# mmailhos/vectorlite

Measured on AMD Instinct MI355X. Metric: flat-cosine QPS @ N=10M dim=384 k=10; achieved HBM GB/s vs peak, higher is better.
Workload: dtype f32; 1 GPU; flat cosine single-query search, N=10000000, dim=384, k=10; rows=10000000, dim=384, k=10, metric=cosine, parallelism=1 GPU

## Files before the change

### vectorlite_amd/csrc/kernels.hip

```cpp
#include "kernels.hpp"
#include "device_common.hpp"
#include "scan_stream.hpp"
#include "score_bound.hpp"

#include <math.h>
#include <stdlib.h>
#include <string.h>

#include <mutex>
#include <tuple>
#include <type_traits>

namespace vl {
using namespace dev;
static_assert(BOUND_COSINE == COSINE && BOUND_EUCLIDEAN == EUCLIDEAN && BOUND_MANHATTAN == MANHATTAN && BOUND_DOT == DOT,
              "score_bound.hpp carries the metric codes of kernels.hpp");
namespace {

template <typename K, typename C>
__global__ __launch_bounds__(1024) void k_merge_lists(const C* __restrict__ lists, int n_lists, size_t in_stride_q,
                                                      C* __restrict__ out, size_t out_stride_q)
{
    constexpr int NW = 16;
    __shared__ C sh[NW * WAVE];
// ... 367 lines not shown
    {
        const uint32_t first = blockIdx.y * QB;
        q64 += (size_t)first * dim;
        out += (size_t)first * gridDim.x * KP;
        n_q = n_q - first < (uint32_t)QB ? n_q - first : (uint32_t)QB;
    }

    for (uint32_t idx = threadIdx.x; idx < QB * LD4; idx += 256) {
        const uint32_t qi = idx / LD4, j = idx % LD4;
        f32x4 z = {0.0f, 0.0f, 0.0f, 0.0f};
        qs[qi][j] = qi < n_q ? load_q4(q64 + (size_t)qi * dim, j, dim) : z;
    }
    __syncthreads();

    const uint32_t n_steps = (n + RPS - 1) / RPS;
    const uint32_t n_waves = gridDim.x * 4;

    TopList<float> L[QB];
    uint32_t n_buf[QB];
#pragma unroll
    for (int qi = 0; qi < QB; ++qi) {
        L[qi].init();
        n_buf[qi] = 0;
    }
    auto flush = [&](int qi) {
        float fk = -INFINITY;
        uint32_t fp = POS_SENTINEL;
        asm volatile("" : "+v"(fk));
        if ((uint32_t)lane < n_buf[qi]) {
            const Cand32 e = cbuf[wave][qi][lane];
            fk = e.key;
            fp = e.pos;
        }
        sort64_reversed<float>(fk, fp);
        L[qi].merge_reversed(fk, fp);
        n_buf[qi] = 0;
    };

    for (uint32_t s = blockIdx.x * 4 + wave; s < n_steps; s += n_waves) {
        const uint32_t row = s * RPS + g;
        const bool valid = row < n;
        const uint32_t r = valid ? row : n - 1;
        const f32x4* p = slab + (size_t)r * LD4 + c;
        f32x4 x[VPL];
#pragma unroll
        for (int j = 0; j < VPL; ++j) x[j] = __builtin_nontemporal_load(p + G * j);
        float inv = 1.0f;
        if (METRIC == COSINE) inv = inv_norm[r];
#pragma unroll
        for (int qi = 0; qi < QB; ++qi) {
            float a = 0.0f;
#pragma unroll
            for (int j = 0; j < VPL; ++j) a = acc4<METRIC>(a, x[j], qs[qi][c + G * j]);
            a = group_reduce<G>(a);
#ifndef VL_DBG_K3_NOINSERT
            {
                const float key = scan_key<METRIC>(a, inv);
                const bool cand = valid && c == 0 && (uint32_t)qi < n_q && better<float>(key, row, L[qi].thr_key, L[qi].thr_pos);
                const unsigned long long m = __ballot(cand);
                if (m != 0ull) {
                    const uint32_t slot = n_buf[qi] + __builtin_amdgcn_mbcnt_hi((uint32_t)(m >> 32), __builtin_amdgcn_mbcnt_lo((uint32_t)m, 0u));
                    if (cand) {
                        Cand32 e;
                        e.key = key;
                        e.pos = row;
                        cbuf[wave][qi][slot] = e;
                    }
                    n_buf[qi] += (uint32_t)__popcll(m);
                    if (n_buf[qi] > (uint32_t)(WAVE - RPS)) flush(qi);
                }
            }
#else
            if (scan_key<METRIC>(a, inv) == 12345.678f) L[qi].pos = row;
#endif
            __builtin_amdgcn_sched_barrier(0);
        }
    }

#pragma unroll
    for (int qi = 0; qi < QB; ++qi) {
        if ((uint32_t)qi < n_q) {
            if (n_buf[qi]) flush(qi);
            block_merge<float, Cand32, 4>(L[qi], sh);
            if (wave == 0) {
                Cand32 e;
                e.key = L[qi].key;
                e.pos = L[qi].pos;
                out[((size_t)qi * gridDim.x + blockIdx.x) * KP + lane] = e;
            }
            __syncthreads();
        }
    }
}

constexpr int RESCORE_CH = 96;

template <int METRIC, int NTHREADS>
__device__ __forceinline__ void rescore_rows(const double* __restrict__ master, const double* __restrict__ q64,
                                             uint32_t dim, const uint32_t* sh_pos, int n_rows,
                                             double (*tile)[RESCORE_CH + 1], double* qtile, Acc64<METRIC>& A)
{
    constexpr int PER = (KP * RESCORE_CH + NTHREADS - 1) / NTHREADS;
    constexpr int PF = (NTHREADS >= 1024) ? 4 : 1;
    const int tid = threadIdx.x;
    A.init();
    if (n_rows <= 0) return;
    for (uint32_t g0 = 0; g0 < dim; g0 += PF * RESCORE_CH) {
        double pre[PF][PER];
        double qpre[PF];
#pragma unroll
        for (int p = 0; p < PF; ++p) {
            const uint32_t c0 = g0 + p * RESCORE_CH;
#pragma unroll
            for (int i = 0; i < PER; ++i) {
                int idx = tid + i * NTHREADS;
                idx = idx < KP * RESCORE_CH ? idx : KP * RESCORE_CH - 1;
                int r = idx / RESCORE_CH;
                r = r < n_rows ? r : n_rows - 1;
                uint32_t col = c0 + (uint32_t)(idx % RESCORE_CH);
                col = col < dim ? col : dim - 1;
                pre[p][i] = master[(size_t)sh_pos[r] * dim + col];
            }
            {
                uint32_t col = c0 + (uint32_t)(tid % RESCORE_CH);
                col = col < dim ? col : dim - 1;
                qpre[p] = q64[col];
            }
        }
#pragma unroll
        for (int p = 0; p < PF; ++p) {
            const uint32_t c0 = g0 + p * RESCORE_CH;
            if (c0 >= dim) break;
            const uint32_t cw = (dim - c0) < (uint32_t)RESCORE_CH ? (dim - c0) : (uint32_t)RESCORE_CH;
            __syncthreads();
#pragma unroll
            for (int i = 0; i < PER; ++i) {
                const int idx = tid + i * NTHREADS;
                if (idx < KP * RESCORE_CH) tile[idx / RESCORE_CH][idx % RESCORE_CH] = pre[p][i];
            }
            if (tid < RESCORE_CH) qtile[tid] = qpre[p];
            __syncthreads();
            if (tid < n_rows) {
                uint32_t cc = 0;
                for (; cc + 8 <= cw; cc += 8) {
                    double xv[8], yv[8];
#pragma unroll
                    for (int t = 0; t < 8; ++t) {
                        xv[t] = tile[tid][cc + t];
                        yv[t] = qtile[cc + t];
                    }
#pragma unroll
                    for (int t = 0; t < 8; ++t) A.step(xv[t], yv[t]);
                }
                for (; cc < cw; ++cc) A.step(tile[tid][cc], qtile[cc]);
            }
        }
    }
}

#ifdef VL_DBG_STAMPS
__device__ unsigned long long vl_dbg_stamps[32];
#define VL_STAMP(i)                                                                  \
    do {                                                                             \
        if (threadIdx.x == 0 && blockIdx.x == 0) {                                   \
            vl_dbg_stamps[i] = __builtin_amdgcn_s_memrealtime();                     \
            vl_dbg_stamps[16 + (i)] = __builtin_amdgcn_s_memtime();  \
        }                                                                            \
    } while (0)
#else
#define VL_STAMP(i) do {} while (0)
#endif

constexpr int RP_CH = 48;
constexpr int RP_NCH = 8;
constexpr int RP_BW = RP_CH * RP_NCH;

template <int METRIC, int ROWS = KP, int NCH = RP_NCH>
struct RescoreLds {
    double tA[ROWS][RP_CH + 1];
    double tB[METRIC == COSINE ? ROWS : 1][RP_CH + 1];
    double qblk[RP_CH * NCH];
    double qq[METRIC == COSINE ? RP_CH * NCH : 1];
    double b[ROWS];
    double c;
};

template <int METRIC, int ROWS, int NTHREADS, int NCH = RP_NCH>
__device__ __forceinline__ void rescore_rows_par(const double* __restrict__ master, const double* __restrict__ q64,
                                                 uint32_t dim, const uint32_t* sh_pos, int n_rows,
                                                 RescoreLds<METRIC, ROWS, NCH>& S, Acc64<METRIC>& A,
                                                 const double (&q_first)[(RP_CH * NCH + NTHREADS - 1) / NTHREADS])
{
    constexpr int RP_PER = ROWS * RP_CH / NTHREADS;
    constexpr int BW = RP_CH * NCH;
    constexpr int QN = (BW + NTHREADS - 1) / NTHREADS;
    static_assert(ROWS * RP_CH % NTHREADS == 0 && ROWS <= WAVE, "tile elements divide evenly; one lane per row");
    const int tid = threadIdx.x;
    const int lane = tid & (WAVE - 1), wave = tid >> 6;
    A.init();
    if (n_rows <= 0) return;
    double acc = (METRIC == COSINE) ? 0.0 : -0.0;
    for (uint32_t g0 = 0; g0 < dim; g0 += BW) {
        double pre[NCH][RP_PER];
#pragma unroll
        for (int p = 0; p < NCH; ++p) {
            const uint32_t c0 = g0 + p * RP_CH;
#pragma unroll
            for (int i = 0; i < RP_PER; ++i) {
                const int idx = tid + i * NTHREADS;
                int r = idx / RP_CH;
                r = r < n_rows ? r : n_rows - 1;
                uint32_t col = c0 + (uint32_t)(idx % RP_CH);
                col = col < dim ? col : dim - 1;
                pre[p][i] = master[(size_t)sh_pos[r] * dim + col];
            }
        }
        double qv[QN];
#pragma unroll
        for (int j = 0; j < QN; ++j) {
            qv[j] = q_first[j];
            if (g0 != 0 && tid + j * NTHREADS < BW) {
                const uint32_t col = g0 + (uint32_t)(tid + j * NTHREADS);
                qv[j] = q64[col < dim ? col : dim - 1];
            }
        }
        VL_STAMP(4);
        __syncthreads();
#pragma unroll
        for (int j = 0; j < QN; ++j)
            if (tid + j * NTHREADS < BW) {
                S.qblk[tid + j * NTHREADS] = qv[j];
                if (METRIC == COSINE) S.qq[tid + j * NTHREADS] = qv[j] * qv[j];
            }
        __syncthreads();
        VL_STAMP(5);
#pragma unroll
        for (int p = 0; p < NCH; ++p) {
            const uint32_t c0 = g0 + p * RP_CH;
            if (c0 >= dim) break;
            const uint32_t cw = (dim - c0) < (uint32_t)RP_CH ? (dim - c0) : (uint32_t)RP_CH;
            if (p) __syncthreads();
#pragma unroll
            for (int i = 0; i < RP_PER; ++i) {
                const int idx = tid + i * NTHREADS;
                const int r = idx / RP_CH, cc = idx % RP_CH;
                const double x = pre[p][i], y = S.qblk[p * RP_CH + cc];
                if (METRIC == COSINE) {
                    S.tA[r][cc] = x * y;
                    S.tB[r][cc] = x * x;
                } else if (METRIC == EUCLIDEAN) {
                    const double d = x - y;
                    S.tA[r][cc] = d * d;
                } else if (METRIC == MANHATTAN) {
                    S.tA[r][cc] = fabs(x - y);
                } else {
                    S.tA[r][cc] = x * y;
                }
            }
            __syncthreads();
            if (wave == 0 || (METRIC == COSINE && wave == 1)) {
                if (lane < n_rows) {
                    const double* t = (wave == 0) ? &S.tA[lane][0] : &S.tB[METRIC == COSINE ? lane : 0][0];
                    uint32_t cc = 0;
                    for (; cc + 16 <= cw; cc += 16) {
                        double v[16];
#pragma unroll
                        for (int u = 0; u < 16; ++u) v[u] = t[cc + u];
#pragma unroll
                        for (int u = 0; u < 16; ++u) acc += v[u];
                    }
                    for (; cc < cw; ++cc) acc += t[cc];
                }
            } else if (METRIC == COSINE && wave == 2) {
                const double* t = &S.qq[p * RP_CH];
                uint32_t cc = 0;
                for (; cc + 16 <= cw; cc += 16) {
                    double v[16];
#pragma unroll
                    for (int u = 0; u < 16; ++u) v[u] = t[cc + u];
#pragma unroll
                    for (int u = 0; u < 16; ++u) acc += v[u];
                }
                for (; cc < cw; ++cc) acc += t[cc];
            }
            if (p == 0) VL_STAMP(6);
        }
    }
    VL_STAMP(7);
    __syncthreads();
    if (METRIC == COSINE) {
        if (wave == 1 && lane < ROWS) S.b[lane] = acc;
        if (wave == 2 && lane == 0) S.c = acc;
        __syncthreads();
        if (wave == 0) {
            A.a = acc;
            A.b = S.b[lane < ROWS ? lane : 0];
            A.c = S.c;
        }
    } else if (wave == 0) {
        A.a = acc;
    }
}


template <int METRIC>
__device__ __forceinline__ void rank_check_emit(double sc, uint32_t my_pos, float key64, int n_cand, uint32_t k, uint64_t n_rows,
                                                uint32_t ld, double R, double Q, double in_extra,
                                                SearchResultBlock* __restrict__ out, uint32_t seq, const ShardRecordSink& sink,
                                                uint32_t q_in_launch)
{
    const int lane = lane_id();
    const bool valid = lane < n_cand;
    const bool any_nan = __ballot(valid && sc != sc) != 0ull;
    int rank = 0;
    for (int j = 0; j < n_cand; ++j) {
        const double sj = read_lane(sc, j);
        const uint32_t pj = read_lane(my_pos, j);
        rank += (sj > sc || (sj == sc && pj < my_pos)) ? 1 : 0;
    }
    const uint32_t k_eff = (uint64_t)k < n_rows ? k : (uint32_t)n_rows;
    uint32_t flags = 0;
    if (any_nan) flags |= RESULT_HAS_NAN | RESULT_NEEDS_EXACT;
    if (n_rows <= (uint64_t)KP) {
        if ((uint64_t)n_cand < n_rows) flags |= RESULT_NEEDS_EXACT;
    } else {
        if (n_cand < KP) {
            flags |= RESULT_NEEDS_EXACT;
        } else {
            const double B = bound_for_key<METRIC>(key64, ld, R, Q, in_extra);
            const unsigned long long at_cut = __ballot(valid && rank == (int)k_eff - 1);
            double s_cut = 0.0;
            if (at_cut) s_cut = __shfl(sc, __ffsll((long long)at_cut) - 1);
            if (!at_cut || !(s_cut > B)) flags |= RESULT_NEEDS_EXACT;
        }
    }
    if (valid && rank < (int)k_eff) {
        out->pos[rank] = my_pos;
        out->score[rank] = sc;
    }
    if (lane == 0) {
        out->n_out = k_eff;
        out->flags = flags;
    }
    if (sink.cnt) {
        const uint32_t q = sink.q0 + q_in_launch;
        const uint32_t offered = (flags == 0u) ? (k_eff < sink.ks ? k_eff : sink.ks) : 0u;
        if (valid && (uint32_t)rank < offered) {
            const size_t e = (size_t)q * sink.ks + (uint32_t)rank;
            sink.score_bits[e] = (unsigned long long)__double_as_longlong(sc);
            sink.gpos[e] = sink.row_offset + (unsigned long long)my_pos;
            sink.ids[e] = sink.pos_to_id[my_pos];
        }
        if (lane == 0) sink.cnt[q] = offered;
    }
    VL_STAMP(9);
    if (seq) {
        __threadfence_system();
        if (lane == 0) __hip_atomic_store(&out->seq, seq, __ATOMIC_RELEASE, __HIP_MEMORY_SCOPE_SYSTEM);
    }
    VL_STAMP(10);
}

constexpr int BF_ROWS = 16;
#ifndef VL_BF_NCH
#define VL_BF_NCH 4
#endif
constexpr int BF_NCH = VL_BF_NCH;
template <int METRIC>
__global__ __launch_bounds__(256) void k_batch_rescore(const Cand32* __restrict__ lists, const double* __restrict__ master,
                                                       const double* __restrict__ q64, uint32_t dim, double* __restrict__ scores)
{
    const uint32_t q = blockIdx.x >> 2, quarter = blockIdx.x & 3u;
    __shared__ RescoreLds<METRIC, BF_ROWS, BF_NCH> rs;
    __shared__ uint32_t sh_pos[BF_ROWS];
    __shared__ int sh_n;
    const int tid = threadIdx.x, lane = tid & (WAVE - 1), wave = tid >> 6;
    const Cand32* mine = lists + (size_t)q * KP + quarter * BF_ROWS;
    q64 += (size_t)q * dim;
    constexpr int QN = (RP_CH * BF_NCH + 255) / 256;
    double q_first[QN];
#pragma unroll
    for (int j = 0; j < QN; ++j) {
        const uint32_t c = (uint32_t)(tid + j * 256);
        q_first[j] = q64[c < dim ? c : dim - 1];
    }
    if (wave == 0) {
        const uint32_t p = lane < BF_ROWS ? mine[lane].pos : POS_SENTINEL;
        if (lane < BF_ROWS) sh_pos[lane] = p;
        const unsigned long long real = __ballot(p != POS_SENTINEL);
        if (lane == 0) sh_n = __popcll(real);
    }
    __syncthreads();
    const int n_mine = sh_n;
    Acc64<METRIC> A;
    rescore_rows_par<METRIC, BF_ROWS, 256, BF_NCH>(master, q64, dim, sh_pos, n_mine, rs, A, q_first);
    if (wave == 0 && lane < BF_ROWS) scores[(size_t)q * KP + quarter * BF_ROWS + lane] = lane < n_mine ? A.score() : 0.0;
}

template <int METRIC>
__global__ __launch_bounds__(256) void k_batch_rank_emit(const Cand32* __restrict__ lists, const double* __restrict__ scores,
                                                         const double* __restrict__ q_norms, uint32_t nq, uint32_t ld,
                                                         uint64_t n_rows, uint32_t k, double R, double in_extra,
                                                         SearchResultBlock* __restrict__ out, ShardRecordSink sink)
{
    const int lane = lane_id();
    const uint32_t q = blockIdx.x * 4 + (threadIdx.x >> 6);
    if (q >= nq) return;
    const Cand32 e = lists[(size_t)q * KP + lane];
    const int n_cand = __popcll(__ballot(e.pos != POS_SENTINEL));
    const double sc = lane < n_cand ? scores[(size_t)q * KP + lane] : 0.0;
    rank_check_emit<METRIC>(sc, e.pos, read_lane(e.key, KP - 1), n_cand, k, n_rows, ld, R, q_norms[q], in_extra, out + q, 0u, sink, q);
}

template <int METRIC>
__global__ __launch_bounds__(1024) void k_merge_finalize(const Cand32* __restrict__ partials, int n_lists,
                                                         size_t list_stride_q, const double* __restrict__ master,
                                                         const double* __restrict__ q64,
                                                         const double* __restrict__ q_norms, uint32_t dim,
                                                         uint32_t ld, uint64_t n_rows, uint32_t k, double R,
                                                         double in_extra, SearchResultBlock* __restrict__ out,
                                                         uint32_t seq, ShardRecordSink sink)
{
    partials += (size_t)blockIdx.x * list_stride_q;
    q64 += (size_t)blockIdx.x * dim;
    out += blockIdx.x;
    const double Q = q_norms[blockIdx.x];
    constexpr int NW = 16;
    __shared__ Cand32 sh_lists[NW * WAVE];
    __shared__ RescoreLds<METRIC> rs;
    __shared__ uint32_t sh_pos[KP];
    __shared__ float sh_key[KP];
    __shared__ int sh_ncand;

    const int lane = lane_id();
    const int wave = threadIdx.x >> 6;

    VL_STAMP(0);
    TopList<float> L;
    double q_first[1] = {0.0};
    {
        const int first = wave * 4;
        int count = n_lists - first;
        count = count < 0 ? 0 : (count > 4 ? 4 : count);
        Cand32 e[4];
        fold_lists4_load<Cand32>(e, partials, first, count);
        if (threadIdx.x < RP_BW) q_first[0] = q64[threadIdx.x < dim ? threadIdx.x : dim - 1];
        fold_lists4_merge<float, Cand32>(L, e, count);
    }
    VL_STAMP(1);
    block_merge_n<float, Cand32>(L, sh_lists, (n_lists + 3) / 4);
    VL_STAMP(2);
    if (wave == 0) {
        sh_pos[lane] = L.pos;
        sh_key[lane] = L.key;
        const unsigned long long real = __ballot(L.pos != POS_SENTINEL);
        if (lane == 0) sh_ncand = __popcll(real);
    }
    __syncthreads();
    const int n_cand = sh_ncand;

    Acc64<METRIC> A;
    VL_STAMP(3);
    rescore_rows_par<METRIC, KP, 1024>(master, q64, dim, sh_pos, n_cand, rs, A, q_first);
    VL_STAMP(8);

    if (wave == 0) {
        const bool valid = lane < n_cand;
        const double sc = valid ? A.score() : 0.0;
        rank_check_emit<METRIC>(sc, sh_pos[lane], sh_key[KP - 1], n_cand, k, n_rows, ld, R, Q, in_extra, out, seq, sink, blockIdx.x);
    }
}

template <int METRIC>
__global__ __launch_bounds__(1024) void k_merge_finalize_jobs(const Cand32* __restrict__ partials, int n_lists,
                                                              size_t list_stride_q, const double* __restrict__ master,
                                                              const double* __restrict__ q64,
                                                              const double* __restrict__ q_norms, uint32_t dim, uint32_t ld,
                                                              const SubsetJobDev* __restrict__ jobs, double R,
                                                              SearchResultBlock* __restrict__ out)
{
    partials += (size_t)blockIdx.x * list_stride_q;
    q64 += (size_t)blockIdx.x * dim;
    out += blockIdx.x;
    const double Q = q_norms[blockIdx.x];
    const SubsetJobDev job = jobs[blockIdx.x];
    constexpr int NW = 16;
    __shared__ Cand32 sh_lists[NW * WAVE];
    __shared__ RescoreLds<METRIC> rs;
    __shared__ uint32_t sh_pos[KP];
    __shared__ float sh_key[KP];
    __shared__ int sh_ncand;

    const int lane = lane_id();
    const int wave = threadIdx.x >> 6;

    TopList<float> L;
    double q_first[1] = {0.0};
    {
        const int first = wave * 4;
        int count = n_lists - first;
        count = count < 0 ? 0 : (count > 4 ? 4 : count);
        Cand32 e[4];
        fold_lists4_load<Cand32>(e, partials, first, count);
        if (threadIdx.x < RP_BW) q_first[0] = q64[threadIdx.x < dim ? threadIdx.x : dim - 1];
        fold_lists4_merge<float, Cand32>(L, e, count);
    }
    block_merge_n<float, Cand32>(L, sh_lists, (n_lists + 3) / 4);
    if (wave == 0) {
        sh_pos[lane] = L.pos;
        sh_key[lane] = L.key;
        const unsigned long long real = __ballot(L.pos != POS_SENTINEL);
        if (lane == 0) sh_ncand = __popcll(real);
    }
    __syncthreads();
    const int n_cand = sh_ncand;

    Acc64<METRIC> A;
    rescore_rows_par<METRIC, KP, 1024>(master, q64, dim, sh_pos, n_cand, rs, A, q_first);

    if (wave == 0) {
        const bool valid = lane < n_cand;
        const double sc = valid ? A.score() : 0.0;
        rank_check_emit<METRIC>(sc, sh_pos[lane], sh_key[KP - 1], n_cand, job.k, (uint64_t)job.m, ld, R, Q, 0.0, out, 0u,
                                ShardRecordSink{}, blockIdx.x);
    }
}

constexpr int KMULTI_PARTS = 4;

template <int METRIC>
__global__ __launch_bounds__(1024) void k_merge_finalize_multi(const Cand32* __restrict__ lists, int n_lists,
                                                               size_t part_stride, int n_parts,
                                                               const double* __restrict__ master,
                                                               const double* __restrict__ q64,
                                                               const double* __restrict__ q_norms, uint32_t dim,
                                                               uint32_t ld, uint64_t n_rows, uint32_t k, double R,
                                                               SearchResultBlock* __restrict__ out)
{
    constexpr int NW = 16;
    __shared__ Cand32 sh_lists[NW * WAVE];
    __shared__ RescoreLds<METRIC> rs;
    __shared__ uint32_t sh_pos[KMULTI_PARTS * KP];
    __shared__ float sh_key[KMULTI_PARTS * KP];
    __shared__ double sh_score[KMULTI_PARTS * KP];
    __shared__ int sh_ncand[KMULTI_PARTS];
    __shared__ int sh_flags;
    __shared__ double sh_cut;
    __shared__ int sh_has_cut;
    const double Q = q_norms[0];
    const int lane = lane_id();
    const int wave = threadIdx.x >> 6;
    double q_first[1] = {0.0};
    if (threadIdx.x < RP_BW) q_first[0] = q64[threadIdx.x < dim ? threadIdx.x : dim - 1];
    if (threadIdx.x == 0) {
        sh_flags = 0;
        sh_has_cut = 0;
        sh_cut = 0.0;
    }
    for (int p = 0; p < n_parts; ++p) {
        TopList<float> L;
        const int first = wave * 4;
        int count = n_lists - first;
        count = count < 0 ? 0 : (count > 4 ? 4 : count);
        fold_lists4<float, Cand32>(L, lists + (size_t)p * part_stride, first, count);
        block_merge<float, Cand32, NW>(L, sh_lists);
        if (wave == 0) {
            sh_pos[p * KP + lane] = L.pos;
            sh_key[p * KP + lane] = L.key;
            const unsigned long long real = __ballot(L.pos != POS_SENTINEL);
            if (lane == 0) sh_ncand[p] = __popcll(real);
        }
        __syncthreads();
    }
    for (int p = 0; p < n_parts; ++p) {
        Acc64<METRIC> A;
        rescore_rows_par<METRIC, KP, 1024>(master, q64, dim, sh_pos + p * KP, sh_ncand[p], rs, A, q_first);
        if (wave == 0) sh_score[p * KP + lane] = lane < sh_ncand[p] ? A.score() : 0.0;
        __syncthreads();
    }
    const int t = threadIdx.x;
    const int total_slots = n_parts * KP;
    const bool valid = t < total_slots && (t % KP) < sh_ncand[t / KP];
    const double sc = valid ? sh_score[t] : 0.0;
    const uint32_t my_pos = t < total_slots ? sh_pos[t] : POS_SENTINEL;
    if (valid && sc != sc) atomicOr(&sh_flags, (int)(RESULT_HAS_NAN | RESULT_NEEDS_EXACT));
    int rank = 0;
    for (int j = 0; j < total_slots; ++j) {
        if ((j % KP) >= sh_ncand[j / KP]) continue;
        const double sj = sh_score[j];
        const uint32_t pj = sh_pos[j];
        rank += (sj > sc || (sj == sc && pj < my_pos)) ? 1 : 0;
    }
    const uint32_t k_eff = (uint64_t)k < n_rows ? k : (uint32_t)n_rows;
    if (valid && rank == (int)k_eff - 1) {
        sh_cut = sc;
        sh_has_cut = 1;
    }
    __syncthreads();
    if (valid && rank < (int)k_eff) {
        out[rank / KP].pos[rank % KP] = my_pos;
        out[rank / KP].score[rank % KP] = sc;
    }
    if (t == 0) {
        uint32_t flags = (uint32_t)sh_flags;
        int total = 0;
        double B = -1.0e300;
        bool excluded_rows = false;
        for (int p = 0; p < n_parts; ++p) {
            total += sh_ncand[p];
            if (sh_ncand[p] == KP) {
                excluded_rows = true;
                const double bp = bound_for_key<METRIC>(sh_key[p * KP + KP - 1], ld, R, Q, 0.0);
                B = bp > B ? bp : B;
            }
        }
        if (!sh_has_cut || (uint32_t)total < k_eff) flags |= RESULT_NEEDS_EXACT;
        else if (excluded_rows && !(sh_cut > B)) flags |= RESULT_NEEDS_EXACT;
        if ((uint64_t)total < n_rows && !excluded_rows) flags |= RESULT_NEEDS_EXACT;
        out[0].n_out = k_eff;
        out[0].flags = flags;
    }
}

constexpr int EX_ROWS = 256;
constexpr int EX_CH = 16;

template <int METRIC>
__global__ __launch_bounds__(256) void k_exact_scan(const double* __restrict__ master,
                                                    const double* __restrict__ q64, uint64_t n, uint32_t dim,
                                                    double* __restrict__ scores, uint32_t* __restrict__ nan_flag)
{
    __shared__ double tile[EX_ROWS][EX_CH + 1];
    __shared__ double qtile[EX_CH];
    const int tid = threadIdx.x;
    const uint64_t n_tiles = (n + EX_ROWS - 1) / EX_ROWS;
    const uint32_t n_chunks = (dim + EX_CH - 1) / EX_CH;
    for (uint64_t t = blockIdx.x; t < n_tiles; t += gridDim.x) {
        const uint64_t row0 = t * EX_ROWS;
        const uint64_t rows_here = (n - row0) < (uint64_t)EX_ROWS ? (n - row0) : (uint64_t)EX_ROWS;
        Acc64<METRIC> A;
        A.init();
        double pre[EX_CH];
        double qpre = 0.0;
        auto fetch = [&](uint32_t c0) {
            const uint32_t cw = (dim - c0) < (uint32_t)EX_CH ? (dim - c0) : (uint32_t)EX_CH;
#pragma unroll
            for (int i = 0; i < EX_CH; ++i) {
                const int idx = tid + i * 256;
                uint64_t r = (uint64_t)(idx / EX_CH);
                uint32_t cc = (uint32_t)(idx % EX_CH);
                r = r < rows_here ? r : rows_here - 1;
                cc = cc < cw ? cc : cw - 1;
                pre[i] = master[(row0 + r) * dim + c0 + cc];
            }
            {
                uint32_t qc = (uint32_t)(tid % EX_CH);
                qc = qc < cw ? qc : cw - 1;
                qpre = q64[c0 + qc];
            }
        };
        fetch(0);
        for (uint32_t ch = 0; ch < n_chunks; ++ch) {
            const uint32_t c0 = ch * EX_CH;
            const uint32_t cw = (dim - c0) < (uint32_t)EX_CH ? (dim - c0) : (uint32_t)EX_CH;
            __syncthreads();
#pragma unroll
            for (int i = 0; i < EX_CH; ++i) {
                const int idx = tid + i * 256;
                tile[idx / EX_CH][idx % EX_CH] = pre[i];
            }
            if (tid < EX_CH) qtile[tid] = qpre;
            __syncthreads();
            if (ch + 1 < n_chunks) fetch(c0 + EX_CH);
            if ((uint64_t)tid < rows_here) {
                if (cw == (uint32_t)EX_CH) {
#pragma unroll
                    for (uint32_t cc = 0; cc < (uint32_t)EX_CH; ++cc) A.step(tile[tid][cc], qtile[cc]);
                } else {
                    for (uint32_t cc = 0; cc < cw; ++cc) A.step(tile[tid][cc], qtile[cc]);
                }
            }
        }
        if ((uint64_t)tid < rows_here) {
            const double sc = A.score();
            scores[row0 + tid] = sc;
            if (sc != sc) atomicOr(nan_flag, 1u);
        }
    }
}

template <int METRIC>
__device__ __forceinline__ void exact_scan_subset_body(const double* __restrict__ master, const double* __restrict__ q64,
                                                       const uint32_t* __restrict__ plist, uint64_t m, uint32_t dim,
                                                       double* __restrict__ scores, uint32_t* __restrict__ nan_flag)
{
    __shared__ double tile[EX_ROWS][EX_CH + 1];
    __shared__ double qtile[EX_CH];
    const int tid = threadIdx.x;
    const uint64_t n_tiles = (m + EX_ROWS - 1) / EX_ROWS;
    const uint32_t n_chunks = (dim + EX_CH - 1) / EX_CH;
    for (uint64_t t = blockIdx.x; t < n_tiles; t += gridDim.x) {
        const uint64_t row0 = t * EX_ROWS;
        const uint64_t rows_here = (m - row0) < (uint64_t)EX_ROWS ? (m - row0) : (uint64_t)EX_ROWS;
        uint64_t src[EX_CH];
#pragma unroll
        for (int i = 0; i < EX_CH; ++i) {
            uint64_t r = (uint64_t)((tid + i * 256) / EX_CH);
            r = r < rows_here ? r : rows_here - 1;
            src[i] = (uint64_t)plist[row0 + r] * dim;
        }
        Acc64<METRIC> A;
        A.init();
        double pre[EX_CH];
        double qpre = 0.0;
        auto fetch = [&](uint32_t c0) {
            const uint32_t cw = (dim - c0) < (uint32_t)EX_CH ? (dim - c0) : (uint32_t)EX_CH;
#pragma unroll
            for (int i = 0; i < EX_CH; ++i) {
                uint32_t cc = (uint32_t)((tid + i * 256) % EX_CH);
                cc = cc < cw ? cc : cw - 1;
                pre[i] = master[src[i] + c0 + cc];
            }
            {
                uint32_t qc = (uint32_t)(tid % EX_CH);
                qc = qc < cw ? qc : cw - 1;
                qpre = q64[c0 + qc];
            }
        };
        fetch(0);
        for (uint32_t ch = 0; ch < n_chunks; ++ch) {
            const uint32_t c0 = ch * EX_CH;
            const uint32_t cw = (dim - c0) < (uint32_t)EX_CH ? (dim - c0) : (uint32_t)EX_CH;
            __syncthreads();
#pragma unroll
            for (int i = 0; i < EX_CH; ++i) {
                const int idx = tid + i * 256;
                tile[idx / EX_CH][idx % EX_CH] = pre[i];
            }
            if (tid < EX_CH) qtile[tid] = qpre;
            __syncthreads();
            if (ch + 1 < n_chunks) fetch(c0 + EX_CH);
            if ((uint64_t)tid < rows_here) {
                if (cw == (uint32_t)EX_CH) {
#pragma unroll
                    for (uint32_t cc = 0; cc < (uint32_t)EX_CH; ++cc) A.step(tile[tid][cc], qtile[cc]);
                } else {
                    for (uint32_t cc = 0; cc < cw; ++cc) A.step(tile[tid][cc], qtile[cc]);
                }
            }
        }
        if ((uint64_t)tid < rows_here) {
            const double sc = A.score();
            scores[row0 + tid] = sc;
            if (sc != sc) atomicOr(nan_flag, 1u);
        }
    }
}

template <int METRIC>
__global__ __launch_bounds__(256) void k_exact_scan_subset(const double* __restrict__ master,
                                                           const double* __restrict__ q64,
                                                           const uint32_t* __restrict__ plist, uint64_t m, uint32_t dim,
                                                           double* __restrict__ scores, uint32_t* __restrict__ nan_flag)
{
    exact_scan_subset_body<METRIC>(master, q64, plist, m, dim, scores, nan_flag);
}

template <int METRIC>
__global__ __launch_bounds__(256) void k_range_rescore(const double* __restrict__ master, const double* __restrict__ q64,
                                                       const uint32_t* __restrict__ cand, uint32_t cap, uint32_t dim,
                                                       double* __restrict__ scores, uint32_t* __restrict__ ctr)
{
    const uint32_t m = ctr[RANGE_CTR_APPENDED];
    if (m == 0 || m > cap) return;
    exact_scan_subset_body<METRIC>(master, q64, cand, (uint64_t)m, dim, scores, ctr + RANGE_CTR_NAN);
}

__global__ __launch_bounds__(256) void k_select64(const double* __restrict__ scores, uint32_t n,
                                                  const SearchResultBlock* __restrict__ after,
                                                  Cand64* __restrict__ out)
{
    __shared__ Cand64 sh[4 * WAVE];
    const int lane = lane_id();
    const int wave = threadIdx.x >> 6;
    const uint32_t n_steps = (n + WAVE - 1) / WAVE;
    const uint32_t n_waves = gridDim.x * 4;
    TopList<double> L;
    L.init();
    const bool cut = after != nullptr;
    const double cut_key = cut ? after->score[KP - 1] : 0.0;
    const uint32_t cut_pos = cut ? after->pos[KP - 1] : 0u;
    for (uint32_t s = blockIdx.x * 4 + wave; s < n_steps; s += n_waves) {
        const uint32_t row = s * WAVE + lane;
        bool valid = row < n;
        const double sc = valid ? scores[row] : 0.0;
        if (cut) valid = valid && better<double>(cut_key, cut_pos, sc, row);
        L.offer(sc, row, valid);
    }
    block_merge<double, Cand64, 4>(L, sh);
    if (wave == 0) {
        Cand64 e;
        e.key = L.key;
        e.pos = L.pos;
        e.pad = 0;
        out[(size_t)blockIdx.x * KP + lane] = e;
    }
}

__global__ __launch_bounds__(1024) void k_merge64_emit(const Cand64* __restrict__ partials, int n_lists,
                                                       uint64_t n_rows, uint32_t k,
                                                       const uint32_t* __restrict__ nan_flag,
                                                       SearchResultBlock* __restrict__ out)
{
    constexpr int NW = 16;
    __shared__ Cand64 sh[NW * WAVE];
    const int lane = lane_id();
    const int wave = threadIdx.x >> 6;
    TopList<double> L;
    {
        const int first = wave * 4;
        int count = n_lists - first;
        count = count < 0 ? 0 : (count > 4 ? 4 : count);
        fold_lists4<double, Cand64>(L, partials, first, count);
    }
    block_merge<double, Cand64, NW>(L, sh);
    if (wave == 0) {
        const uint32_t k_eff = (uint64_t)k < n_rows ? k : (uint32_t)n_rows;
        if ((uint32_t)lane < k_eff || k == (uint32_t)KP) {
            out->pos[lane] = L.pos;
            out->score[lane] = L.key;
        }
        if (lane == 0) {
            out->n_out = k_eff;
            out->flags = (*nan_flag) ? RESULT_HAS_NAN : 0u;
        }
    }
}

__device__ __forceinline__ unsigned long long desc_key(double s)
{
    s = s + 0.0;
    unsigned long long b = (unsigned long long)__double_as_longlong(s);
    const unsigned long long asc = (b >> 63) ? ~b : (b | 0x8000000000000000ull);
    return ~asc;
}

__global__ void k_sort_init(const double* __restrict__ scores, uint64_t n, uint64_t cap,
                            unsigned long long* __restrict__ okeys, uint32_t* __restrict__ opos)
{
    for (uint64_t i = blockIdx.x * (uint64_t)blockDim.x + threadIdx.x; i < cap;
         i += (uint64_t)gridDim.x * blockDim.x) {
        if (i < n) {
            okeys[i] = desc_key(scores[i]);
            opos[i] = (uint32_t)i;
        } else {
            okeys[i] = ~0ull;
            opos[i] = POS_SENTINEL;
        }
    }
}

template <typename P>
__device__ __forceinline__ bool pair_greater(unsigned long long ka, P pa, unsigned long long kb, P pb)
{
    return ka > kb || (ka == kb && pa > pb);
}

constexpr int SORT_LOCAL = 2048;
static_assert((uint32_t)SORT_LOCAL == RANGE_SMALL, "a range search's speculative ranking is one local sort");

template <typename P>
__global__ __launch_bounds__(1024) void k_bitonic_local(unsigned long long* __restrict__ okeys, P* __restrict__ opos,
                                                        uint64_t k_lo, uint64_t k_hi)
{
    __shared__ unsigned long long sk[SORT_LOCAL];
    __shared__ P sp[SORT_LOCAL];
    const uint64_t base = (uint64_t)blockIdx.x * SORT_LOCAL;
    const int tid = threadIdx.x;
    sk[tid] = okeys[base + tid];
// ... 1170 lines not shown
```

Baseline: 1587 queries/s.

## Replace block-parallel rescore with chunked double-buffered single-pass rescore

After: 1571 queries/s. No clear change (-1.0%).

```diff
diff --git a/vectorlite_amd/csrc/kernels.hip b/vectorlite_amd/csrc/kernels.hip
--- a/vectorlite_amd/csrc/kernels.hip
+++ b/vectorlite_amd/csrc/kernels.hip
@@ -693,6 +693,143 @@
     }
 }
 
+constexpr int RS_CH = 64;
+constexpr int RS_NCH = RP_BW / RS_CH;
+static_assert(RS_CH * RS_NCH == RP_BW, "the callers fetch the query's first RP_BW columns");
+
+template <int METRIC>
+struct RescoreLds1 {
+    double tA[2][KP][RS_CH + 1];
+    double tB[METRIC == COSINE ? 2 : 1][METRIC == COSINE ? KP : 1][RS_CH + 1];
+    double qblk[RP_BW];
+    double qq[METRIC == COSINE ? RP_BW : 1];
+    double b[KP];
+    double c;
+};
+
+template <int METRIC>
+__device__ __forceinline__ void rescore_rows_single(const double* __restrict__ master, const double* __restrict__ q64,
+                                                    uint32_t dim, const uint32_t* sh_pos, int n_rows,
+                                                    RescoreLds1<METRIC>& S, Acc64<METRIC>& A, const double (&q_first)[1])
+{
+    constexpr int NTHREADS = 1024;
+    constexpr int PER = KP * RS_CH / NTHREADS;
+    const int tid = threadIdx.x;
+    const int lane = tid & (WAVE - 1), wave = tid >> 6;
+    A.init();
+    if (n_rows <= 0) return;
+    double acc = (METRIC == COSINE) ? 0.0 : -0.0;
+    for (uint32_t g0 = 0; g0 < dim; g0 += RP_BW) {
+        double pre[RS_NCH][PER];
+#pragma unroll
+        for (int p = 0; p < RS_NCH; ++p) {
+            uint32_t col = g0 + p * RS_CH + (uint32_t)lane;
+            col = col < dim ? col : dim - 1;
+#pragma unroll
+            for (int i = 0; i < PER; ++i) {
+                int r = wave + i * (NTHREADS / RS_CH);
+                r = r < n_rows ? r : n_rows - 1;
+                pre[p][i] = master[(size_t)sh_pos[r] * dim + col];
+            }
+        }
+        double qv = q_first[0];
+        if (g0 != 0 && tid < RP_BW) {
+            const uint32_t col = g0 + (uint32_t)tid;
+            qv = q64[col < dim ? col : dim - 1];
+        }
+        VL_STAMP(4);
+        __syncthreads();
+        if (tid < RP_BW) {
+            S.qblk[tid] = qv;
+            if (METRIC == COSINE) S.qq[tid] = qv * qv;
+        }
+        __syncthreads();
+        VL_STAMP(5);
+        auto produce = [&](int p) {
+#pragma unroll
+            for (int i = 0; i < PER; ++i) {
+                const int r = wave + i * (NTHREADS / RS_CH);
+                const double x = pre[p][i], y = S.qblk[p * RS_CH + lane];
+                if (METRIC == COSINE) {
+                    S.tA[p & 1][r][lane] = x * y;
+                    S.tB[METRIC == COSINE ? (p & 1) : 0][METRIC == COSINE ? r : 0][lane] = x * x;
+                } else if (METRIC == EUCLIDEAN) {
+                    const double d = x - y;
+                    S.tA[p & 1][r][lane] = d * d;
+                } else if (METRIC == MANHATTAN) {
+                    S.tA[p & 1][r][lane] = fabs(x - y);
+                } else {
+                    S.tA[p & 1][r][lane] = x * y;
+                }
+            }
+        };
+        produce(0);
+#pragma unroll
+        for (int p = 0; p < RS_NCH; ++p) {
+            const uint32_t c0 = g0 + p * RS_CH;
+            if (c0 >= dim) break;
+            const uint32_t cw = (dim - c0) < (uint32_t)RS_CH ? (dim - c0) : (uint32_t)RS_CH;
+            __syncthreads();
+            const double* t = &S.tA[p & 1][lane][0];
+            bool walk = wave == 0 && lane < n_rows;
+            if (METRIC == COSINE && wave == 1) {
+                t = &S.tB[METRIC == COSINE ? (p & 1) : 0][METRIC == COSINE ? lane : 0][0];
+                walk = lane < n_rows;
+            }
+            if (METRIC == COSINE && wave == 2) {
+                t = &S.qq[p * RS_CH];
+                walk = true;
+            }
+            constexpr int RB = 8;
+            const bool full = cw == (uint32_t)RS_CH;
+            double v[2][RB];
+            if (walk && full) {
+#pragma unroll
+                for (int u = 0; u < RB; ++u) v[0][u] = t[u];
+            }
+            __builtin_amdgcn_sched_barrier(0);
+            if (p + 1 < RS_NCH && c0 + RS_CH < dim) produce(p + 1);
+            __builtin_amdgcn_sched_barrier(0);
+            if (walk && full) {
+#pragma unroll
+                for (int g = 0; g < RS_CH / RB; ++g) {
+                    if (g + 1 < RS_CH / RB) {
+#pragma unroll
+                        for (int u = 0; u < RB; ++u) v[(g + 1) & 1][u] = t[(g + 1) * RB + u];
+                    }
+#pragma unroll
+                    for (int u = 0; u < RB; ++u) acc += v[g & 1][u];
+                }
+            } else if (walk) {
+                uint32_t cc = 0;
+                for (; cc + RB <= cw; cc += RB) {
+                    double w[RB];
+#pragma unroll
+                    for (int u = 0; u < RB; ++u) w[u] = t[cc + u];
+#pragma unroll
+                    for (int u = 0; u < RB; ++u) acc += w[u];
+                }
+                for (; cc < cw; ++cc) acc += t[cc];
+            }
+            if (p == 0) VL_STAMP(6);
+        }
+    }
+    VL_STAMP(7);
+    __syncthreads();
+    if (METRIC == COSINE) {
+        if (wave == 1) S.b[lane] = acc;
+        if (wave == 2 && lane == 0) S.c = acc;
+        __syncthreads();
+        if (wave == 0) {
+            A.a = acc;
+            A.b = S.b[lane];
+            A.c = S.c;
+        }
+    } else if (wave == 0) {
+        A.a = acc;
+    }
+}
+
 
 template <int METRIC>
 __device__ __forceinline__ void rank_check_emit(double sc, uint32_t my_pos, float key64, int n_cand, uint32_t k, uint64_t n_rows,
@@ -818,7 +955,7 @@
     const double Q = q_norms[blockIdx.x];
     constexpr int NW = 16;
     __shared__ Cand32 sh_lists[NW * WAVE];
-    __shared__ RescoreLds<METRIC> rs;
+    __shared__ RescoreLds1<METRIC> rs;
     __shared__ uint32_t sh_pos[KP];
     __shared__ float sh_key[KP];
     __shared__ int sh_ncand;
@@ -852,7 +989,7 @@
 
     Acc64<METRIC> A;
     VL_STAMP(3);
-    rescore_rows_par<METRIC, KP, 1024>(master, q64, dim, sh_pos, n_cand, rs, A, q_first);
+    rescore_rows_single<METRIC>(master, q64, dim, sh_pos, n_cand, rs, A, q_first);
     VL_STAMP(8);
 
     if (wave == 0) {
@@ -877,7 +1014,7 @@
     const SubsetJobDev job = jobs[blockIdx.x];
     constexpr int NW = 16;
     __shared__ Cand32 sh_lists[NW * WAVE];
-    __shared__ RescoreLds<METRIC> rs;
+    __shared__ RescoreLds1<METRIC> rs;
     __shared__ uint32_t sh_pos[KP];
     __shared__ float sh_key[KP];
     __shared__ int sh_ncand;
@@ -907,7 +1044,7 @@
     const int n_cand = sh_ncand;
 
     Acc64<METRIC> A;
-    rescore_rows_par<METRIC, KP, 1024>(master, q64, dim, sh_pos, n_cand, rs, A, q_first);
+    rescore_rows_single<METRIC>(master, q64, dim, sh_pos, n_cand, rs, A, q_first);
 
     if (wave == 0) {
         const bool valid = lane < n_cand;
@@ -930,7 +1067,7 @@
 {
     constexpr int NW = 16;
     __shared__ Cand32 sh_lists[NW * WAVE];
-    __shared__ RescoreLds<METRIC> rs;
+    __shared__ RescoreLds1<METRIC> rs;
     __shared__ uint32_t sh_pos[KMULTI_PARTS * KP];
     __shared__ float sh_key[KMULTI_PARTS * KP];
     __shared__ double sh_score[KMULTI_PARTS * KP];
@@ -965,7 +1102,7 @@
     }
     for (int p = 0; p < n_parts; ++p) {
         Acc64<METRIC> A;
-        rescore_rows_par<METRIC, KP, 1024>(master, q64, dim, sh_pos + p * KP, sh_ncand[p], rs, A, q_first);
+        rescore_rows_single<METRIC>(master, q64, dim, sh_pos + p * KP, sh_ncand[p], rs, A, q_first);
         if (wave == 0) sh_score[p * KP + lane] = lane < sh_ncand[p] ? A.score() : 0.0;
         __syncthreads();
     }
```
